# goalheart/ionic-mpnn

Measured on AMD Instinct MI355X. Metric: molecule-graph pairs/sec (fwd), batch 4096 per MI355X, higher is better.
Workload: dtype f32 (bf16x9 emulation)

## Files before the change

ionic_mpnn_amd/csrc/encoder_layout.h:

```cpp
#pragma once

#include "common.h"

namespace impnn {
namespace enc {

typedef float f32x4 __attribute__((ext_vector_type(4)));
typedef _Float16 half8 __attribute__((ext_vector_type(8)));

constexpr float kSW = 256.0f;
constexpr float kSX = 16.0f;
constexpr float kAcc = kSW * kSX;

constexpr int kD = 32;
constexpr int kKMax = 8;
constexpr int kRCap = 256;
constexpr int kECap = 1024;
constexpr int kHS = 36;
constexpr int kMsgRS = 36;
constexpr int kUpdRS = 68;
constexpr int kThreads = 1024;
constexpr int kWaves = kThreads / 64;
constexpr int kTbCapFloats = 2048;

__host__ __device__ constexpr int img_msg_floats(int K) { return K * kD * kMsgRS; }
__host__ __device__ constexpr int img_upd_floats() { return 3 * kD * kUpdRS; }
__host__ __device__ constexpr int img_vec_floats() { return 5 * kD; }
__host__ __device__ constexpr int img_floats(int K) {
  return img_msg_floats(K) + img_upd_floats() + img_vec_floats();
}
__host__ __device__ constexpr int img16_msg_halfs(int K) { return K * 2 * 2 * 512; }
__host__ __device__ constexpr int img16_upd_halfs() { return 3 * 2 * 2 * 2 * 512; }
__host__ __device__ constexpr int img16_vec_float_off(int K) { return (img16_msg_halfs(K) + img16_upd_halfs()) / 2; }
__host__ __device__ constexpr int feat_of(int q, int j) { return 16 * (j >> 2) + 4 * q + (j & 3); }
constexpr int kPf = 4;
constexpr int kImgSlot = kPf * kThreads * 4;
static_assert(kThreads == 4 * kRCap, "prologue maps 4 threads to a row");
static_assert(img_floats(kKMax) <= kImgSlot, "weight image does not fit its slot");
static_assert(img16_vec_float_off(kKMax) + img_vec_floats() <= kImgSlot, "split weight image does not fit");

constexpr int kRecRowptr = 0;
constexpr int kRecTilemax = 528;
constexpr int kRecMoloff = 544;
constexpr int kRecMolrows = 1072;
constexpr int kRecPoolrow = 1584;
constexpr int kRecRowatom = 2096;
constexpr int kEntMaxAtom = 454;
constexpr int kRecEnt = 3136;
constexpr int kRecBytes = 8192;
static_assert(kRecEnt + 4 * kECap <= kRecBytes && kRecEnt % 16 == 0, "record layout");

constexpr int kTECap = 512;
constexpr int kTECapBig = 640;
__host__ __device__ constexpr int tecap_of(int E) { return E > kTECap ? kTECapBig : kTECap; }
constexpr int kTVbMax = 256;
constexpr int kTHS = 36;
constexpr int kTAS = 32;
constexpr int kTRecRowdeg = 0;
constexpr int kTRecTilemax = 528;
constexpr int kTRecMoloff = 544;
constexpr int kTRecMolrows = 1072;
constexpr int kTRecPoolrow = 1584;
constexpr int kTRecRowatom = 2096;
constexpr int kTRecCounts = 3120;
constexpr int kTRecJdptr = 3136;
constexpr int kTRecNrun = 3664;
constexpr int kTRecGrp = 3712;
constexpr int kTRunTarget = 32;
__host__ __device__ constexpr int tgrp_cap(int Vb, int ecap) { return ecap / 4 + (Vb < kTVbMax ? Vb : kTVbMax); }
__host__ __device__ constexpr int trec_runs_off(int Vb, int ecap) { return kTRecGrp + 16 * tgrp_cap(Vb, ecap); }
__host__ __device__ constexpr int trec_used_bytes(int Vb, int ecap) {
  return (trec_runs_off(Vb, ecap) + 2 * (Vb + 2 + kTRunTarget) + 15) & ~15;
}
constexpr int kTRecBytes = 12288;
constexpr int kTRecPart1 = 8192;
__host__ __device__ constexpr int trec_lds_bytes(int Vb, int ecap) { return trec_used_bytes(Vb, ecap); }
static_assert(kTRecGrp % 16 == 0 && trec_used_bytes(kTVbMax, kTECapBig) <= kTRecBytes, "typed record layout");
__host__ __device__ constexpr int tmsg_floats(int ecap) { return (ecap + 2) * kD; }
__host__ __device__ constexpr int tmsg_off(int s, int u) { return s * kD + ((u ^ ((s >> 1) & 7)) << 2); }
__host__ __device__ constexpr int tmsg_key(int s) { return s * kD + (((s >> 1) & 7) << 2); }
static_assert(tmsg_key(kTECapBig + 1) < 65536, "message keys travel as 16 bits");
constexpr int kTUpdBlocks = 24;
constexpr int kTVecFloatOff = kTUpdBlocks * 256;
constexpr int kTUpdFloats = kTVecFloatOff + 5 * kD;
constexpr int kTUpdSlot = 2 * kThreads * 4;
constexpr int kTUpdLds = 6400;
static_assert(kTUpdFloats <= kTUpdLds && kTUpdLds <= kTUpdSlot, "typed update image");
constexpr int kXUpdHalfs = 3 * 2 * 2 * 3 * 512;
constexpr int kXVecFloatOff = kXUpdHalfs / 2;
constexpr int kXUpdFloats = kXVecFloatOff + 5 * kD;
constexpr int kXUpdSlot = 3 * kThreads * 4;
constexpr int kXUpdLds = 9472;
static_assert(kXUpdFloats <= kXUpdLds && kXUpdLds <= kXUpdSlot, "x3 update image");
constexpr int kTMatFloats = kD * kD;
inline size_t typed_prepared_floats(int S, int Vb, bool x3 = false) {
  const size_t s = S > 0 ? S : 1;
  return s * (x3 ? kXUpdSlot : kTUpdSlot) + s * (size_t)Vb * kTMatFloats + (size_t)Vb * kTMatFloats;
}

constexpr int kShareCap = kECap;
inline int plan_vmin(int n_ions, int B, int vrmax, int nwg) {
  const int64_t span = 2 * (int64_t)n_ions * B * vrmax / (nwg > 0 ? nwg : 1) + vrmax;
  const int64_t v = (span + kShareCap - 2) / (kShareCap - 1);
  return (int)(v < 1 ? 1 : (v > kRCap ? kRCap : v));
}
constexpr int kMaxHops = 128;

constexpr int kPB = 16;

struct Ws {
  size_t img_off, rows_off, vr_off, partial_off, share_off, nsub_off, desc_off, rec_off, total;
  int nwg;
  int max_sub;
  int nblk;
  int rec_bytes;
};

inline size_t align_up(size_t x, size_t a) { return (x + a - 1) / a * a; }

__host__ __device__ constexpr int tvr_of_edges(int edges, int ecap) { return (edges * kRCap + ecap - 1) / ecap; }

inline int vr_max_of(int N, int E, bool typed = false) {
  int v = typed ? (E > 4 * kTECapBig ? kRCap + 1 : tvr_of_edges(E, tecap_of(E))) : (E + 3) / 4;
  int m = N > v ? N : v;
  m = m < 1 ? 1 : m;
  return typed && m > kRCap ? kRCap : m;
}

struct PlanHeader {
  int32_t magic, kind, n_ions, B, N, E, nwg, max_sub;
  int32_t overflow;
};
constexpr int32_t kPlanMagic = 0x696d706e;
constexpr int32_t kPlanBadBit = 1 << 30;

inline Ws ws_layout(int n_ions, int B, int N, int E, int S, int Vb, int nwg, bool typed, bool x3 = false) {
  Ws w{};
  const int vrmax = vr_max_of(N, E, typed);
  w.rec_bytes = typed ? kTRecBytes : kRecBytes;
  const int win = kRCap - vrmax + 1;
  w.nwg = nwg;
  w.nblk = (B + kPB - 1) / kPB;
  const int64_t share_rows = (2 * (int64_t)n_ions * B * vrmax) / nwg + vrmax;
  const int64_t by_win = win >= 1 ? share_rows / win + 2 : (int64_t)1 << 40;
  const int64_t by_pairs = 2 * share_rows / (kRCap + 1) + 2;
  w.max_sub = (int)(by_win < by_pairs ? by_win : by_pairs);
  size_t off = 256;
  w.img_off = off;
  off = align_up(off + (typed ? (size_t)n_ions * typed_prepared_floats(S, Vb, x3)
                              : (size_t)n_ions * (S > 0 ? S : 1) * kImgSlot) * sizeof(float), 256);
  w.rows_off = off;
  off = align_up(off + (size_t)n_ions * B * sizeof(int32_t), 256);
  w.vr_off = off;
  off = align_up(off + (size_t)n_ions * B * sizeof(int32_t), 256);
  w.partial_off = off;
  off = align_up(off + (size_t)n_ions * w.nblk * sizeof(int32_t), 256);
  w.share_off = off;
  off = align_up(off + (size_t)nwg * 4 * sizeof(int32_t), 256);
  w.nsub_off = off;
  off = align_up(off + (size_t)nwg * sizeof(int32_t), 256);
// ... 101 lines not shown
```

ionic_mpnn_amd/csrc/encoder_plan.hip:

```cpp
#include "encoder_layout.h"

namespace impnn {
namespace enc {

namespace {

__global__ __launch_bounds__(64 * kPB) void plan_stats_kernel(PlanParams p) {
  __shared__ int vsum[kPB], vbad[kPB];
  __builtin_amdgcn_s_setprio(3);
  const int lane = threadIdx.x & 63, wv = threadIdx.x >> 6;
  const int g = blockIdx.x / p.nblk, blk = blockIdx.x - g * p.nblk;
  const int b = blk * kPB + wv;
  const bool have = b < p.B;
  const int64_t item = (int64_t)g * p.B + (have ? b : 0);
  int my_vr = 0, my_bad = 0;
  if (have) {
  const int32_t* ids = p.atom_ids[g] + (int64_t)b * p.N;
  const int32_t* cn = p.conn[g] + (int64_t)b * p.E * 2;
  const int32_t* bd = p.bond_ids[g] + (int64_t)b * p.E;
  int rmax = 0, cnt = 0;
  const int id_first = lane < p.N ? ids[lane] : 0;
  int emax = 0;
  for (int e0 = 0; e0 < p.E; e0 += 256) {
    int2 st[4];
// ... 798 lines not shown
        if (ce >= E) { ce -= E; ++cm; }
        const int mo = moloff[m < M ? m : 0];
        row[k] = mo + (ok ? sst[k0 + k].y : 0);
        srw[k] = mo + (ok ? sst[k0 + k].x : 0);
      }
#pragma unroll
      for (int k = 0; k < 3; ++k) {
        const bool ok = (okm >> (k0 + k)) & 1u;
        tk[k] = atomicAdd(&cnt[ok ? row[k] : kRCap + lane], 1);
        atomicAdd(&thist[ok ? sbid[k0 + k] : kTVbMax + lane], 1);
      }
#pragma unroll
      for (int k = 0; k < 3; ++k) {
        const bool ok = (okm >> (k0 + k)) & 1u;
        if (ok && tk[k] < kTick) tick[row[k] * kTick + tk[k]] = (uint16_t)es[k];
        if (ok) {
          if (pos < kTECapBig)
            elist[pos] = make_uint2((uint32_t)row[k] | ((uint32_t)srw[k] << 8) | ((uint32_t)sbid[k0 + k] << 16), (uint32_t)es[k]);
          ++pos;
        }
      }
    }
  }
  for (int s0 = kSC * kRCap; s0 < n_slots; s0 += kRCap) {
    const int slot = s0 + tid;
    int2 st = make_int2(0, 0);
    int bid = -1;
    if (slot < n_slots) {
      st = *reinterpret_cast<const int2*>(conn_c + 2 * (int64_t)slot);
      bid = bond_c[slot];
    }
    const bool ok = edge_valid(st.x, st.y, bid, N, p.Vb);
    const int m = fast_div(slot, E, rE), e = slot - m * E;
    const int mo = moloff[m < M ? m : 0];
    const int row = mo + (ok ? st.y : 0);
    int tk = kTick;
    if (ok) {
      tk = atomicAdd(&cnt[row], 1);
      atomicAdd(&thist[bid], 1);
    }
    const unsigned long long okb = __ballot(ok);
    int pos0 = 0;
    if (okb != 0ull) {
      if (lane == (int)__builtin_ctzll(okb)) pos0 = atomicAdd(&misc[1], (int)__builtin_popcountll(okb));
      pos0 = __builtin_amdgcn_readlane(pos0, (int)__builtin_ctzll(okb));
    }
    if (tk < kTick) tick[row * kTick + tk] = (uint16_t)e;
    const int pos = pos0 + (int)__builtin_popcountll(okb & ((1ull << lane) - 1));
    if (ok && pos < kTECapBig)
      elist[pos] = make_uint2((uint32_t)row | ((uint32_t)(mo + st.x) << 8) | ((uint32_t)bid << 16), (uint32_t)e);
  }
  lds_barrier();
  CSTAMP(3);

  const int my_deg = cnt[tid];
  const int dcl = my_deg > 255 ? 255 : my_deg;
  if (tid < R) {
    if (my_deg > 255) p.header->overflow = 1;
    atomicAdd(&dbins[255 - dcl], 1);
  }
  lds_barrier();
  CSTAMP(4);

  if (wave == 0) {
    const int4 h = reinterpret_cast<const int4*>(dbins)[lane];
    const int s4 = h.x + h.y + h.z + h.w;
    const int ex = wave_incl_scan(s4) - s4;
    reinterpret_cast<int4*>(dstart)[lane] = make_int4(ex, ex + h.x, ex + h.x + h.y, ex + h.x + h.y + h.z);
    __builtin_amdgcn_s_waitcnt(0xc07f);
    const int4 s = reinterpret_cast<const int4*>(dstart)[63 - lane];
    const int t4 = s.x + s.y + s.z + s.w;
    const int incl = wave_incl_scan(t4);
    const int jx = incl - t4;
    reinterpret_cast<int4*>(jdp)[lane] = make_int4(jx, jx + s.w, jx + s.w + s.z, jx + s.w + s.z + s.y);
    if (lane == 63) { jdp[kRCap] = incl; jdp[kRCap + 1] = incl; }
  } else if (wave == 1) {
    const int4 n = reinterpret_cast<const int4*>(thist)[lane];
    const int4 ng = make_int4((n.x + 3) >> 2, (n.y + 3) >> 2, (n.z + 3) >> 2, (n.w + 3) >> 2);
    const int s4 = ng.x + ng.y + ng.z + ng.w;
    const int incl = wave_incl_scan(s4);
    const int ex = incl - s4;
    reinterpret_cast<int4*>(tgb)[lane] = make_int4(ex, ex + ng.x, ex + ng.x + ng.y, ex + ng.x + ng.y + ng.z);
    const int ngrp_all = __builtin_amdgcn_readlane(incl, 63);
    int gmax = (ngrp_all + kTRunTarget - 1) / kTRunTarget;
    gmax = gmax < 2 ? 2 : gmax;
    const float rgm = 1.0f / (float)gmax;
    const int4 nr = make_int4(fast_div(ng.x + gmax - 1, gmax, rgm), fast_div(ng.y + gmax - 1, gmax, rgm),
                              fast_div(ng.z + gmax - 1, gmax, rgm), fast_div(ng.w + gmax - 1, gmax, rgm));
    const int r4 = nr.x + nr.y + nr.z + nr.w;
    const int rincl = wave_incl_scan(r4);
    int ri = rincl - r4;
    uint16_t* runs = reinterpret_cast<uint16_t*>(rec + trec_runs_off(p.Vb, p.ecap));
    for (int i = 0; i < nr.x; ++i) runs[ri++] = (uint16_t)(ex + i * gmax);
    for (int i = 0; i < nr.y; ++i) runs[ri++] = (uint16_t)(ex + ng.x + i * gmax);
    for (int i = 0; i < nr.z; ++i) runs[ri++] = (uint16_t)(ex + ng.x + ng.y + i * gmax);
    for (int i = 0; i < nr.w; ++i) runs[ri++] = (uint16_t)(ex + ng.x + ng.y + ng.z + i * gmax);
    if (lane == 63) {
      runs[rincl] = (uint16_t)incl;
      *reinterpret_cast<uint16_t*>(rec + kTRecNrun) = (uint16_t)rincl;
      misc[0] = incl;
    }
  }
  lds_barrier();
  CSTAMP(5);

  int pos = tid;
  if (tid < R) pos = dstart[255 - dcl] + atomicAdd(&dcur[255 - dcl], 1);
  place[tid] = pos;
  {
    const int my_id = idl[tid];
    r_rowatom[pos] = my_id;
    r_poolrow[tid] = (uint16_t)(pos | (my_id > 0 ? 0x8000 : 0));
    r_rowdeg[pos] = (uint16_t)my_deg;
    if ((pos & 15) == 0) r_tilemax[pos >> 4] = (unsigned char)dcl;
    r_jd[tid] = (uint16_t)jdp[tid];
    if (tid < 2) r_jd[kRCap + tid] = (uint16_t)jdp[kRCap];
    if (pos == 0) {
      r_cw[0] = (uint16_t)misc[0];
      r_cw[1] = (uint16_t)jdp[kRCap];
      r_cw[2] = (uint16_t)dcl;
    }
  }
  {
    const int n_t = thist[tid];
    const int ng = (n_t + 3) >> 2, gb = tgb[tid];
    const uint32_t dump = (uint32_t)tmsg_key(p.ecap) * 0x10001u;
    for (int jg = 0; jg < ng; ++jg) {
      const int c = n_t - 4 * jg;
      grp[gb + jg] = make_uint4((uint32_t)tid | ((uint32_t)(c < 4 ? c : 4) << 8) | ((uint32_t)(ng - jg) << 24), 0u, dump, dump);
    }
  }
  lds_barrier();
  CSTAMP(6);

  {
    auto below = [](uint4 a, uint32_t ue) {
      return (int)(((a.x & 0xffffu) < ue) + ((a.x >> 16) < ue) + ((a.y & 0xffffu) < ue) + ((a.y >> 16) < ue) +
                   ((a.z & 0xffffu) < ue) + ((a.z >> 16) < ue) + ((a.w & 0xffffu) < ue) + ((a.w >> 16) < ue));
    };
    const int nval = misc[1] < kTECapBig ? misc[1] : kTECapBig;
    for (int i0 = 0; i0 < nval; i0 += 2 * kRCap) {
      bool ok[2];
      uint2 en[2];
      int row[2], srow[2], deg[2], ix[2], gb[2], rank[2];
      uint4 ta[2], tb[2];
#pragma unroll
      for (int k = 0; k < 2; ++k) {
        const int i = i0 + k * kRCap + tid;
        ok[k] = i < nval;
        en[k] = elist[ok[k] ? i : 0];
      }
#pragma unroll
      for (int k = 0; k < 2; ++k) {
        const int rt = (int)(en[k].x & 0xffu), bid = (int)(en[k].x >> 16);
        deg[k] = cnt[rt];
        ta[k] = reinterpret_cast<const uint4*>(tick)[2 * rt];
        tb[k] = reinterpret_cast<const uint4*>(tick)[2 * rt + 1];
        row[k] = place[rt];
        srow[k] = place[(en[k].x >> 8) & 0xffu];
        gb[k] = tgb[bid];
        ix[k] = atomicAdd(&tcur[ok[k] ? bid : kTVbMax + lane], 1);
      }
#pragma unroll
      for (int k = 0; k < 2; ++k) {
        rank[k] = below(ta[k], en[k].y) + below(tb[k], en[k].y);
        if (deg[k] > kTick) {
          const int rt = (int)(en[k].x & 0xffu);
          int lo = 0, hi = M - 1;
          while (lo < hi) {
            const int mid = (lo + hi + 1) >> 1;
            if (moloff[mid] <= rt) lo = mid; else hi = mid - 1;
          }
          const int t = rt - moloff[lo];
          const int32_t* cm = conn_c + 2 * (int64_t)lo * E;
          const int32_t* bm = bond_c + (int64_t)lo * E;
          rank[k] = 0;
          for (int e2 = 0; e2 < (int)en[k].y; ++e2) {
            const int2 s2 = *reinterpret_cast<const int2*>(cm + 2 * e2);
            rank[k] += (s2.y == t && edge_valid(s2.x, s2.y, bm[e2], N, p.Vb)) ? 1 : 0;
          }
        }
        rank[k] = jdp[rank[k] < 256 ? rank[k] : 255];
      }
#pragma unroll
      for (int k = 0; k < 2; ++k) {
        if (ok[k]) {
          unsigned char* ge = reinterpret_cast<unsigned char*>(&grp[gb[k] + (ix[k] >> 2)]);
          ge[4 + (ix[k] & 3)] = (unsigned char)srow[k];
          reinterpret_cast<uint16_t*>(ge + 8)[ix[k] & 3] = (uint16_t)tmsg_key(rank[k] + row[k]);
        }
      }
    }
  }
  lds_barrier();
  CSTAMP(9);

  {
    const int ngrp = misc[0];
    uint4* r_grp = reinterpret_cast<uint4*>(rec + kTRecGrp);
    for (int i = tid; i < ngrp; i += kRCap) r_grp[i] = grp[i];
  }
  CSTAMP(15);
  lds_barrier();
// ... 43 lines not shown
```

ionic_mpnn_amd/csrc/encoder_typed.hip:

```cpp
#include "encoder_device.h"
#include "encoder_layout.h"

namespace impnn {
namespace enc {

namespace {

constexpr int kOffUpd = 0;
constexpr int off_h(bool x3) { return kOffUpd + (x3 ? kXUpdLds : kTUpdLds); }
constexpr int kTHSBig3 = 32;
constexpr int off_msg(bool x3, int hs = kTHS) { return off_h(x3) + kRCap * hs; }
constexpr int off_rec(bool x3, int ecap, int hs = kTHS) { return off_msg(x3, hs) + tmsg_floats(ecap); }
constexpr size_t lds_fixed_bytes(bool x3, int Vb, int ecap, int hs = kTHS) {
  return sizeof(float) * (size_t)off_rec(x3, ecap, hs) + trec_lds_bytes(Vb, ecap);
}
static_assert(lds_fixed_bytes(true, kTVbMax, kTECap) <= 160 * 1024 && lds_fixed_bytes(false, kTVbMax, kTECapBig) <= 160 * 1024 &&
                  lds_fixed_bytes(true, kTVbMax, kTECapBig, kTHSBig3) <= 160 * 1024,
              "LDS budget");

typedef __bf16 bf16x8 __attribute__((ext_vector_type(8)));
struct B3 {
  bf16x8 p0, p1, p2;
};
__device__ __forceinline__ void split_pair(float x, float y, unsigned& w0, unsigned& w1, unsigned& w2) {
// ... 2 lines not shown
  const unsigned x1b = __builtin_bit_cast(unsigned, x1), y1b = __builtin_bit_cast(unsigned, y1);
  const float x2 = x1 - __builtin_bit_cast(float, x1b & 0xffff0000u), y2 = y1 - __builtin_bit_cast(float, y1b & 0xffff0000u);
  w0 = __builtin_amdgcn_perm(yb, xb, 0x07060302u);
  w1 = __builtin_amdgcn_perm(y1b, x1b, 0x07060302u);
  w2 = __builtin_amdgcn_perm(__builtin_bit_cast(unsigned, y2), __builtin_bit_cast(unsigned, x2), 0x07060302u);
}
__device__ __forceinline__ B3 split8x3(f32x4 a, f32x4 b) {
  union {
    bf16x8 v;
    unsigned u[4];
  } q0, q1, q2;
  split_pair(a[0], a[1], q0.u[0], q1.u[0], q2.u[0]);
  split_pair(a[2], a[3], q0.u[1], q1.u[1], q2.u[1]);
  split_pair(b[0], b[1], q0.u[2], q1.u[2], q2.u[2]);
  split_pair(b[2], b[3], q0.u[3], q1.u[3], q2.u[3]);
  B3 r;
  r.p0 = q0.v;
  r.p1 = q1.v;
  r.p2 = q2.v;
  return r;
}
__device__ __forceinline__ f32x4 mfmab(bf16x8 a, bf16x8 b, f32x4 c) {
  return __builtin_amdgcn_mfma_f32_16x16x32_bf16(a, b, c, 0, 0, 0);
}
__device__ __forceinline__ void mma9x2(f32x4& c0, f32x4& c1, const __bf16* blk0, const __bf16* blk1, int lane, const B3& b) {
  const bf16x8 a00 = *reinterpret_cast<const bf16x8*>(blk0 + lane * 8);
  const bf16x8 a01 = *reinterpret_cast<const bf16x8*>(blk0 + 512 + lane * 8);
  const bf16x8 a02 = *reinterpret_cast<const bf16x8*>(blk0 + 1024 + lane * 8);
  const bf16x8 a10 = *reinterpret_cast<const bf16x8*>(blk1 + lane * 8);
  const bf16x8 a11 = *reinterpret_cast<const bf16x8*>(blk1 + 512 + lane * 8);
  const bf16x8 a12 = *reinterpret_cast<const bf16x8*>(blk1 + 1024 + lane * 8);
  c0 = mfmab(a02, b.p2, c0);  c1 = mfmab(a12, b.p2, c1);
  c0 = mfmab(a01, b.p2, c0);  c1 = mfmab(a11, b.p2, c1);
  c0 = mfmab(a02, b.p1, c0);  c1 = mfmab(a12, b.p1, c1);
  c0 = mfmab(a00, b.p2, c0);  c1 = mfmab(a10, b.p2, c1);
  c0 = mfmab(a02, b.p0, c0);  c1 = mfmab(a12, b.p0, c1);
  c0 = mfmab(a01, b.p1, c0);  c1 = mfmab(a11, b.p1, c1);
  c0 = mfmab(a00, b.p1, c0);  c1 = mfmab(a10, b.p1, c1);
  c0 = mfmab(a01, b.p0, c0);  c1 = mfmab(a11, b.p0, c1);
  c0 = mfmab(a00, b.p0, c0);  c1 = mfmab(a10, b.p0, c1);
}

template <int ABID>
__device__ __forceinline__ f32x4 mfma1(float a, float b, f32x4 c) {
  return __builtin_amdgcn_mfma_f32_4x4x1f32(a, b, c, 3, ABID, 0);
}

typedef float f32x2v __attribute__((ext_vector_type(2)));
struct Grp {
  uint4 ge;
  f32x2v aq;
};
struct Run {
  f32x4 bq[4];
  Grp first;
};

#ifndef IMPNN_T_PF
#define IMPNN_T_PF 0
#endif
#ifndef IMPNN_T_EARLY
#define IMPNN_T_EARLY 0
#endif
constexpr int kPfWhere = IMPNN_T_PF, kRunsEarly = IMPNN_T_EARLY;

template <bool STAMPS, bool X3, int HS = kTHS>
__global__ __launch_bounds__(kThreads, kThreads / 256) void encoder_typed_kernel(TEncParams p) {
  extern __shared__ __align__(16) float smem[];
  constexpr int kUpdLds = X3 ? kXUpdLds : kTUpdLds, kUpdSlot = X3 ? kXUpdSlot : kTUpdSlot;
  constexpr int kNPf = X3 ? 3 : 2;
  float* const wupd = smem + kOffUpd;
  float* const wvec = wupd + (X3 ? kXVecFloatOff : kTVecFloatOff);
  float* const hbuf = smem + off_h(X3);
  float* const msg = smem + off_msg(X3, HS);
  const int zero_slot = p.ecap + 1;
  unsigned char* const recl = reinterpret_cast<unsigned char*>(smem + off_rec(X3, p.ecap, HS));
  const int rec_lds = p.rec_lds;
  float* const atab = reinterpret_cast<float*>(recl + rec_lds);
  const uint16_t* const r_rowdeg = reinterpret_cast<const uint16_t*>(recl + kTRecRowdeg);
  const unsigned char* const r_tilemax = recl + kTRecTilemax;
  const uint16_t* const r_moloff = reinterpret_cast<const uint16_t*>(recl + kTRecMoloff);
  const uint16_t* const r_molrows = reinterpret_cast<const uint16_t*>(recl + kTRecMolrows);
  const uint16_t* const r_poolrow = reinterpret_cast<const uint16_t*>(recl + kTRecPoolrow);
  const int32_t* const r_rowatom = reinterpret_cast<const int32_t*>(recl + kTRecRowatom);
  const uint16_t* const r_jdptr = reinterpret_cast<const uint16_t*>(recl + kTRecJdptr);
  const uint16_t* const r_runs = reinterpret_cast<const uint16_t*>(recl + trec_runs_off(p.Vb, p.ecap));
  int* const run_ctr = reinterpret_cast<int*>(recl + kTRecCounts + 8);
  const uint4* const r_grp = reinterpret_cast<const uint4*>(recl + kTRecGrp);

  const int tid = threadIdx.x, lane = tid & 63;
  const int wave = __builtin_amdgcn_readfirstlane(tid >> 6);
  const int a = lane & 15, q = lane >> 4;
  unsigned long long* stamp = STAMPS && p.stamps ? p.stamps + (size_t)blockIdx.x * 32 : nullptr;
  if (stamp && tid == 0) stamp[0] = __builtin_amdgcn_s_memtime();

  {
    const PlanHeader hd = *p.header;
    if (hd.magic != kPlanMagic || hd.kind != 1 || hd.nwg != (int)gridDim.x || hd.max_sub != p.max_sub ||
        hd.B != p.B || hd.n_ions != p.n_ions || hd.overflow != 0) {
      const float nan = __builtin_nanf("");
      for (int g = 0; g < p.n_ions; ++g)
        for (int64_t t = (int64_t)blockIdx.x * kThreads + tid; t < (int64_t)p.B * kD; t += (int64_t)gridDim.x * kThreads)
          p.pooled[g][t] = nan;
      return;
    }
  }
  const int c_begin = blockIdx.x * p.max_sub;
  const int c_end = c_begin + __builtin_amdgcn_readfirstlane(p.nsub[blockIdx.x]);
  if (c_begin >= c_end) return;

  if (p.atab_lds)
    for (int t = tid; t < (p.Va + 1) * (kTAS / 4); t += kThreads)
      st4(atab + 4 * t, t < p.Va * (kD / 4) ? ld4(p.atom_table + 4 * t) : f32x4{0.f, 0.f, 0.f, 0.f});
  if (tid < kD) msg[zero_slot * kD + tid] = 0.f;
  unsigned long long t_pro = 0, t_steps = 0, t_pool = 0, t_mark = 0, t_msg = 0;
  if (stamp && tid == 0) t_mark = __builtin_amdgcn_s_memtime();

  auto pool = [&](int M, int m0, int g) {
    float* out_g = p.pooled[g];
    for (int t0 = 0; t0 < M * 64; t0 += kThreads) {
      const int t = t0 + tid;
      const int part = t & 7, f4 = (t >> 3) & 7, m = t >> 6;
      f32x4 acc = {0.f, 0.f, 0.f, 0.f};
      if (m < M) {
        const int nr = r_molrows[m], mo = r_moloff[m];
        for (int n = part; n < nr; n += 8) {
          const int pr = r_poolrow[mo + n];
          if (pr & 0x8000) acc += ld4(hbuf + (pr & 0xff) * HS + 4 * f4);
        }
      }
#pragma unroll
      for (int i = 0; i < 4; ++i) {
        float v = acc[i];
        v += __builtin_bit_cast(float, __builtin_amdgcn_update_dpp(0, __builtin_bit_cast(int, v), 0xb1, 0xf, 0xf, true));
        v += __builtin_bit_cast(float, __builtin_amdgcn_update_dpp(0, __builtin_bit_cast(int, v), 0x4e, 0xf, 0xf, true));
        v += __builtin_bit_cast(float, __builtin_amdgcn_update_dpp(0, __builtin_bit_cast(int, v), 0x141, 0xf, 0xf, true));
        acc[i] = v;
      }
      if (m < M && part == 0) st4(out_g + (int64_t)(m0 + m) * kD + 4 * f4, acc);
    }
  };
  auto fill_h0 = [&]() {
    const int row = tid >> 2, sub = tid & 3;
    const int id = r_rowatom[row];
    f32x4 v0 = {0.f, 0.f, 0.f, 0.f}, v1 = v0;
    if ((unsigned)id < (unsigned)p.Va) {
      if (p.atab_lds) {
        v0 = ld4(atab + id * kTAS + 8 * sub);
        v1 = ld4(atab + id * kTAS + 8 * sub + 4);
      } else {
        v0 = ld4(p.atom_table + (int64_t)id * kD + 8 * sub);
        v1 = ld4(p.atom_table + (int64_t)id * kD + 8 * sub + 4);
      }
    }
    st4(hbuf + row * HS + 8 * sub, v0);
    st4(hbuf + row * HS + 8 * sub + 4, v1);
  };

  if (p.S == 0) {
    for (int c = c_begin; c < c_end; ++c) {
      const unsigned char* rc = p.rec + (size_t)c * kTRecBytes;
      if (8 * tid < rec_lds) reinterpret_cast<uint2*>(recl)[tid] = reinterpret_cast<const uint2*>(rc)[tid];
      const int4 dsc = reinterpret_cast<const int4*>(p.desc)[c];
      lds_barrier();
      fill_h0();
      lds_barrier();
      pool(__builtin_amdgcn_readfirstlane(dsc.y), __builtin_amdgcn_readfirstlane(dsc.x),
           __builtin_amdgcn_readfirstlane(dsc.w) >> 16);
      lds_barrier();
    }
    return;
  }

  const bool rec_big = rec_lds > kTRecPart1;
  const unsigned char* rec_c = p.rec + (size_t)c_begin * kTRecBytes;
  uint2 rec_n8 = reinterpret_cast<const uint2*>(rec_c)[tid];
  uint32_t rec_n4 = rec_big ? reinterpret_cast<const uint32_t*>(rec_c + kTRecPart1)[tid] : 0u;
  int4 dsc_next = reinterpret_cast<const int4*>(p.desc)[c_begin];

  const uint32_t* const grp_x = reinterpret_cast<const uint32_t*>(r_grp);
  const int kh = lane >> 5, f = lane & 31;
  const int boff = kh * 512 + f * 4;
  const int ysh = 8 * (lane & 3), zsh = 16 * kh;
  const int acol = 16 * kh + 2 * ((lane >> 2) & 7);

  for (int c = c_begin; c < c_end; ++c) {
    const int4 dsc = dsc_next;
    const int m0 = __builtin_amdgcn_readfirstlane(dsc.x), M = __builtin_amdgcn_readfirstlane(dsc.y);
    const int rg = __builtin_amdgcn_readfirstlane(dsc.w);
    const int R = rg & 0xffff, g = rg >> 16;
    const int ntiles = (R + 15) >> 4;
    const float* upd_g = p.upd[g];
    const float* tmat_g = p.tmat[g];
    if (8 * tid < rec_lds) reinterpret_cast<uint2*>(recl)[tid] = rec_n8;
    if (rec_big && kTRecPart1 + 4 * tid < rec_lds) reinterpret_cast<uint32_t*>(recl + kTRecPart1)[tid] = rec_n4;
    {
      const int cn = (c + 1) < c_end ? (c + 1) : c;
      const unsigned char* rn = p.rec + (size_t)cn * kTRecBytes;
      rec_n8 = reinterpret_cast<const uint2*>(rn)[tid];
      if (rec_big) rec_n4 = reinterpret_cast<const uint32_t*>(rn + kTRecPart1)[tid];
      dsc_next = reinterpret_cast<const int4*>(p.desc)[cn];
    }
    lds_barrier();
    fill_h0();
    if (tid == 0) *run_ctr = 2 * kWaves;
    lds_barrier();
    if (stamp && tid == 0) {
      const unsigned long long t = __builtin_amdgcn_s_memtime();
      t_pro += t - t_mark;
      t_mark = t;
    }
    const int nrun = __builtin_amdgcn_readfirstlane(*reinterpret_cast<const uint16_t*>(recl + kTRecNrun));

    Run P, Q;
    int gP = 0, nP = 0, gQ = 0, nQ = 0;
    bool haveP = false, haveQ = false;
    const bool sP = wave < nrun, sQ = wave + kWaves < nrun;
    const int sgP = __builtin_amdgcn_readfirstlane(r_runs[sP ? wave : 0]);
    const int snP = __builtin_amdgcn_readfirstlane(r_runs[(sP ? wave : 0) + 1]) - sgP;
    const int sgQ = __builtin_amdgcn_readfirstlane(r_runs[sQ ? wave + kWaves : 0]);
    const int snQ = __builtin_amdgcn_readfirstlane(r_runs[(sQ ? wave + kWaves : 0) + 1]) - sgQ;
    const int soP = sP ? (__builtin_amdgcn_readfirstlane(grp_x[4 * sgP]) & 0xff) * kTMatFloats : 0;
    const int soQ = sQ ? (__builtin_amdgcn_readfirstlane(grp_x[4 * sgQ]) & 0xff) * kTMatFloats : 0;
    const int lboffP = sP ? boff : 0, lboffQ = sQ ? boff : 0;
    f32x4 pf[kNPf];
    auto fetch_pf = [&](int s_) {
#pragma unroll
      for (int i = 0; i < kNPf; ++i) pf[i] = ld4(upd_g + (int64_t)s_ * kUpdSlot + 4 * (tid + i * kThreads));
    };
    auto fetch_P = [&](int s_) {
      const float* tm = tmat_g + (size_t)s_ * p.Vb * kTMatFloats;
#pragma unroll
      for (int i = 0; i < 4; ++i) P.bq[i] = ld4(tm + soP + lboffP + i * 128);
    };
    auto fetch_Q = [&](int s_) {
      const float* tm = tmat_g + (size_t)s_ * p.Vb * kTMatFloats;
#pragma unroll
      for (int i = 0; i < 4; ++i) Q.bq[i] = ld4(tm + soQ + lboffQ + i * 128);
    };
    if (kPfWhere != 0) fetch_pf(0);
    if (kRunsEarly >= 1) fetch_P(0);
    if (kRunsEarly >= 2) fetch_Q(0);
    for (int s = 0; s < p.S; ++s) {
      const float* tm_s = tmat_g + (size_t)s * p.Vb * kTMatFloats;
      __builtin_amdgcn_s_setprio(2);
      {
        const float* const abase = hbuf + acol;
        auto load_group = [&](int e, Grp& G) {
          G.ge = r_grp[e];
          const int src = __builtin_amdgcn_ubfe(G.ge.y, ysh, 8);
          G.aq = *reinterpret_cast<const f32x2v*>(abase + src * HS);
        };
        auto compute = [&](const Grp& G, const f32x4 (&bq)[4]) {
          f32x4 acc0 = {0.f, 0.f, 0.f, 0.f}, acc1 = acc0;
#ifndef IMPNN_DIAG_NO_MSG_MFMA
          acc0 = mfma1<0>(G.aq[0], bq[0][0], acc0);
          acc1 = mfma1<0>(G.aq[1], bq[0][1], acc1);
          acc0 = mfma1<1>(G.aq[0], bq[0][2], acc0);
          acc1 = mfma1<1>(G.aq[1], bq[0][3], acc1);
          acc0 = mfma1<2>(G.aq[0], bq[1][0], acc0);
          acc1 = mfma1<2>(G.aq[1], bq[1][1], acc1);
          acc0 = mfma1<3>(G.aq[0], bq[1][2], acc0);
          acc1 = mfma1<3>(G.aq[1], bq[1][3], acc1);
          acc0 = mfma1<4>(G.aq[0], bq[2][0], acc0);
          acc1 = mfma1<4>(G.aq[1], bq[2][1], acc1);
          acc0 = mfma1<5>(G.aq[0], bq[2][2], acc0);
          acc1 = mfma1<5>(G.aq[1], bq[2][3], acc1);
          acc0 = mfma1<6>(G.aq[0], bq[3][0], acc0);
          acc1 = mfma1<6>(G.aq[1], bq[3][1], acc1);
          acc0 = mfma1<7>(G.aq[0], bq[3][2], acc0);
          acc1 = mfma1<7>(G.aq[1], bq[3][3], acc1);
#else
          acc0[0] = G.aq[0] + bq[0][0] + bq[3][3];
          acc1[1] = G.aq[1] + bq[1][1] + bq[2][2];
#endif
          float x0 = acc0[0] + acc1[0], x1 = acc0[1] + acc1[1], x2 = acc0[2] + acc1[2], x3 = acc0[3] + acc1[3];
          asm volatile("s_nop 1\n\tv_permlane32_swap_b32 %0, %1\n\tv_permlane32_swap_b32 %2, %3"
                       : "+v"(x0), "+v"(x1), "+v"(x2), "+v"(x3));
          msg[__builtin_amdgcn_ubfe(G.ge.z, zsh, 16) ^ f] = x0 + x1;
          msg[__builtin_amdgcn_ubfe(G.ge.w, zsh, 16) ^ f] = x2 + x3;
        };
        auto run_type = [&](int g_, int n_, Run& Rn) {
          const int end = g_ + n_;
          Grp T;
          int e = g_;
          while (true) {
            if (e + 1 < end) load_group(e + 1, T);
            compute(Rn.first, Rn.bq);
            if (++e >= end) break;
            if (e + 1 < end) load_group(e + 1, Rn.first);
            compute(T, Rn.bq);
            if (++e >= end) break;
          }
        };
        auto fetch = [&](bool have, int r, int& g_, int& n_, Run& Rn, const float* tm) {
          const int rc = have ? r : 0;
          g_ = __builtin_amdgcn_readfirstlane(r_runs[rc]);
          n_ = __builtin_amdgcn_readfirstlane(r_runs[rc + 1]) - g_;
          const int type = have ? (__builtin_amdgcn_readfirstlane(grp_x[4 * g_]) & 0xff) : 0;
          const float* bp = tm + (size_t)type * kTMatFloats + (have ? boff : 0);
#pragma unroll
          for (int i = 0; i < 4; ++i) Rn.bq[i] = ld4(bp + i * 128);
        };
        auto next_run = [&]() {
          int r = 0;
          if (lane == 0) r = atomicAdd(run_ctr, 1);
          return __builtin_amdgcn_readfirstlane(r);
        };
        auto take = [&](int r, int& g_, int& n_, Run& Rn) {
          fetch(true, r, g_, n_, Rn, tm_s);
          load_group(g_, Rn.first);
        };
        auto landed = [](f32x4 (&b)[4]) {
          asm volatile("" : "+v"(b[0]), "+v"(b[1]), "+v"(b[2]), "+v"(b[3]) : : "memory");
        };
        if (kPfWhere == 0) fetch_pf(s);
        if (kRunsEarly < 1) fetch_P(s);
        if (kRunsEarly < 2) fetch_Q(s);
        haveP = sP; gP = sgP; nP = snP;
        haveQ = sQ; gQ = sgQ; nQ = snQ;
        if (haveP) load_group(gP, P.first);
        if (haveQ) load_group(gQ, Q.first);
        if (haveP) {
          if (!haveQ) {
            landed(P.bq);
            run_type(gP, nP, P);
          } else {
            while (true) {
              landed(P.bq);
              run_type(gP, nP, P);
              const int rP = next_run();
              if (rP >= nrun) {
                landed(Q.bq);
                run_type(gQ, nQ, Q);
                break;
              }
              take(rP, gP, nP, P);
              landed(Q.bq);
              run_type(gQ, nQ, Q);
              const int rQ = next_run();
              if (rQ >= nrun) {
                landed(P.bq);
                run_type(gP, nP, P);
                break;
              }
              take(rQ, gQ, nQ, Q);
            }
          }
        }
      }
#pragma unroll
      for (int i = 0; i < kNPf; ++i)
        if (4 * (tid + i * kThreads) < kUpdLds) st4(wupd + 4 * (tid + i * kThreads), pf[i]);
      const bool mstamp = stamp && c == c_begin && s == 1;
      if (mstamp && lane == 0) stamp[16 + wave] = __builtin_amdgcn_s_memtime();
      lds_barrier();
      if (tid == 0) *run_ctr = 2 * kWaves;
      if (mstamp && tid == 0) stamp[12] = __builtin_amdgcn_s_memtime();
      if (stamp && tid == 0 && c == c_begin && s == 1) t_msg = __builtin_amdgcn_s_memtime();

      int my_tile = -1;
      {
        const int grp = wave & 3, slot = wave >> 2, q4 = ntiles >> 2, r4 = ntiles & 3;
        const int heavy = (4 - r4) * q4;
        if (grp >= r4) {
          if (slot < q4) my_tile = slot * (4 - r4) + (grp - r4);
        } else if (slot <= q4) {
          my_tile = heavy + slot * r4 + grp;
        }
      }
      const bool has_tile = my_tile >= 0 && my_tile < ntiles;
      if (has_tile) {
        const int tile = my_tile;
        const int row = tile * 16 + a;
        const int deg = r_rowdeg[row];
        const int maxdeg = __builtin_amdgcn_readfirstlane(r_tilemax[tile]);
        f32x4 agg0 = {0.f, 0.f, 0.f, 0.f}, agg1 = agg0;
        for (int d0 = 0; d0 < maxdeg; d0 += 4) {
          const uint2 jd = *reinterpret_cast<const uint2*>(r_jdptr + d0);
          int sl[4];
          sl[0] = d0 + 0 < deg ? (int)(jd.x & 0xffffu) + row : zero_slot;
          sl[1] = d0 + 1 < deg ? (int)(jd.x >> 16) + row : zero_slot;
          sl[2] = d0 + 2 < deg ? (int)(jd.y & 0xffffu) + row : zero_slot;
          sl[3] = d0 + 3 < deg ? (int)(jd.y >> 16) + row : zero_slot;
          f32x4 m0v[4], m1v[4];
#pragma unroll
          for (int j = 0; j < 4; ++j) {
            const int o = tmsg_off(sl[j], q);
            m0v[j] = ld4(msg + o);
            m1v[j] = ld4(msg + (o ^ 16));
          }
#pragma unroll
          for (int j = 0; j < 4; ++j) {
// ... 219 lines not shown
```

Baseline: 35.36 million.

## Pack run entries with type and length, drop rowatom from LDS, pipeline records

Run descriptors become 32-bit entries holding the first group, the matrix type (which doubles as the matrix offset) and the run length. This removes the extra LDS reads of the next run start and of the group header when fetching a run. The row-atom section is no longer copied into LDS; each thread prefetches its atom id from global memory alongside the next record, and the LDS record shrinks by that cut. The run counter is now initialised in the planner, one barrier is removed from the record handoff, and pooling is changed to one molecule per wave with batched loads. The trade-off is tighter bit-field limits, which are checked by static asserts.

```diff
diff --git a/ionic_mpnn_amd/csrc/encoder_layout.h b/ionic_mpnn_amd/csrc/encoder_layout.h
--- a/ionic_mpnn_amd/csrc/encoder_layout.h
+++ b/ionic_mpnn_amd/csrc/encoder_layout.h
@@ -68,14 +68,33 @@
 constexpr int kTRecGrp = 3712;
 constexpr int kTRunTarget = 32;
 __host__ __device__ constexpr int tgrp_cap(int Vb, int ecap) { return ecap / 4 + (Vb < kTVbMax ? Vb : kTVbMax); }
+constexpr int kTRunGrpBits = 10, kTRunTypeBits = 8;
+constexpr uint32_t kTRunGrpMask = (1u << kTRunGrpBits) - 1u;
+constexpr uint32_t kTRunMatMask = ((1u << kTRunTypeBits) - 1u) << kTRunGrpBits;
+constexpr int kTRunLenShift = kTRunGrpBits + kTRunTypeBits;
+__host__ __device__ constexpr int trun_gmax(int groups) {
+  return (groups + kTRunTarget - 1) / kTRunTarget < 2 ? 2 : (groups + kTRunTarget - 1) / kTRunTarget;
+}
+__host__ __device__ constexpr uint32_t trun_entry(int first, int type, int groups) {
+  return (uint32_t)first | ((uint32_t)type << kTRunGrpBits) | ((uint32_t)groups << kTRunLenShift);
+}
+static_assert(tgrp_cap(kTVbMax, kTECapBig) <= (1 << kTRunGrpBits) && kTVbMax <= (1 << kTRunTypeBits) &&
+                  trun_gmax(tgrp_cap(kTVbMax, kTECapBig)) < (1 << (32 - kTRunLenShift)) &&
+                  (1 << kTRunGrpBits) == kD * kD,
+              "run entry fields (the type field doubles as the matrix offset: kTMatFloats = 1 << kTRunGrpBits)");
 __host__ __device__ constexpr int trec_runs_off(int Vb, int ecap) { return kTRecGrp + 16 * tgrp_cap(Vb, ecap); }
 __host__ __device__ constexpr int trec_used_bytes(int Vb, int ecap) {
-  return (trec_runs_off(Vb, ecap) + 2 * (Vb + 2 + kTRunTarget) + 15) & ~15;
+  return (trec_runs_off(Vb, ecap) + 4 * ((Vb < kTVbMax ? Vb : kTVbMax) + kTRunTarget) + 15) & ~15;
 }
 constexpr int kTRecBytes = 12288;
 constexpr int kTRecPart1 = 8192;
-__host__ __device__ constexpr int trec_lds_bytes(int Vb, int ecap) { return trec_used_bytes(Vb, ecap); }
+constexpr int kTRecCut = 4 * kRCap;
+__host__ __device__ constexpr int trec_lds_off(int off) { return off < kTRecRowatom ? off : off - kTRecCut; }
+__host__ __device__ constexpr int trec_lds_bytes(int Vb, int ecap) { return trec_used_bytes(Vb, ecap) - kTRecCut; }
 static_assert(kTRecGrp % 16 == 0 && trec_used_bytes(kTVbMax, kTECapBig) <= kTRecBytes, "typed record layout");
+static_assert(kTRecRowatom % 8 == 0 && kTRecCut % 16 == 0 && kTRecRowatom + kTRecCut <= kTRecCounts &&
+                  kTRecPart1 > kTRecRowatom + kTRecCut,
+              "the cut is a whole number of the copy's 8-byte words, inside the first part of the copy");
 __host__ __device__ constexpr int tmsg_floats(int ecap) { return (ecap + 2) * kD; }
 __host__ __device__ constexpr int tmsg_off(int s, int u) { return s * kD + ((u ^ ((s >> 1) & 7)) << 2); }
 __host__ __device__ constexpr int tmsg_key(int s) { return s * kD + (((s >> 1) & 7) << 2); }
diff --git a/ionic_mpnn_amd/csrc/encoder_plan.hip b/ionic_mpnn_amd/csrc/encoder_plan.hip
--- a/ionic_mpnn_amd/csrc/encoder_plan.hip
+++ b/ionic_mpnn_amd/csrc/encoder_plan.hip
@@ -904,21 +904,25 @@
     const int ex = incl - s4;
     reinterpret_cast<int4*>(tgb)[lane] = make_int4(ex, ex + ng.x, ex + ng.x + ng.y, ex + ng.x + ng.y + ng.z);
     const int ngrp_all = __builtin_amdgcn_readlane(incl, 63);
-    int gmax = (ngrp_all + kTRunTarget - 1) / kTRunTarget;
-    gmax = gmax < 2 ? 2 : gmax;
+    const int gmax = trun_gmax(ngrp_all);
     const float rgm = 1.0f / (float)gmax;
     const int4 nr = make_int4(fast_div(ng.x + gmax - 1, gmax, rgm), fast_div(ng.y + gmax - 1, gmax, rgm),
                               fast_div(ng.z + gmax - 1, gmax, rgm), fast_div(ng.w + gmax - 1, gmax, rgm));
     const int r4 = nr.x + nr.y + nr.z + nr.w;
     const int rincl = wave_incl_scan(r4);
     int ri = rincl - r4;
-    uint16_t* runs = reinterpret_cast<uint16_t*>(rec + trec_runs_off(p.Vb, p.ecap));
-    for (int i = 0; i < nr.x; ++i) runs[ri++] = (uint16_t)(ex + i * gmax);
-    for (int i = 0; i < nr.y; ++i) runs[ri++] = (uint16_t)(ex + ng.x + i * gmax);
-    for (int i = 0; i < nr.z; ++i) runs[ri++] = (uint16_t)(ex + ng.x + ng.y + i * gmax);
-    for (int i = 0; i < nr.w; ++i) runs[ri++] = (uint16_t)(ex + ng.x + ng.y + ng.z + i * gmax);
+    uint32_t* runs = reinterpret_cast<uint32_t*>(rec + trec_runs_off(p.Vb, p.ecap));
+    auto put_runs = [&](int type, int first, int groups, int n) {
+      for (int i = 0; i < n; ++i) {
+        const int left = groups - i * gmax;
+        runs[ri++] = trun_entry(first + i * gmax, type, left < gmax ? left : gmax);
+      }
+    };
+    put_runs(4 * lane + 0, ex, ng.x, nr.x);
+    put_runs(4 * lane + 1, ex + ng.x, ng.y, nr.y);
+    put_runs(4 * lane + 2, ex + ng.x + ng.y, ng.z, nr.z);
+    put_runs(4 * lane + 3, ex + ng.x + ng.y + ng.z, ng.w, nr.w);
     if (lane == 63) {
-      runs[rincl] = (uint16_t)incl;
       *reinterpret_cast<uint16_t*>(rec + kTRecNrun) = (uint16_t)rincl;
       misc[0] = incl;
     }
@@ -941,6 +945,7 @@
       r_cw[0] = (uint16_t)misc[0];
       r_cw[1] = (uint16_t)jdp[kRCap];
       r_cw[2] = (uint16_t)dcl;
+      *reinterpret_cast<int32_t*>(rec + kTRecCounts + 8) = 2 * kWaves;
     }
   }
   {
diff --git a/ionic_mpnn_amd/csrc/encoder_typed.hip b/ionic_mpnn_amd/csrc/encoder_typed.hip
--- a/ionic_mpnn_amd/csrc/encoder_typed.hip
+++ b/ionic_mpnn_amd/csrc/encoder_typed.hip
@@ -108,11 +108,10 @@
   const uint16_t* const r_moloff = reinterpret_cast<const uint16_t*>(recl + kTRecMoloff);
   const uint16_t* const r_molrows = reinterpret_cast<const uint16_t*>(recl + kTRecMolrows);
   const uint16_t* const r_poolrow = reinterpret_cast<const uint16_t*>(recl + kTRecPoolrow);
-  const int32_t* const r_rowatom = reinterpret_cast<const int32_t*>(recl + kTRecRowatom);
-  const uint16_t* const r_jdptr = reinterpret_cast<const uint16_t*>(recl + kTRecJdptr);
-  const uint16_t* const r_runs = reinterpret_cast<const uint16_t*>(recl + trec_runs_off(p.Vb, p.ecap));
-  int* const run_ctr = reinterpret_cast<int*>(recl + kTRecCounts + 8);
-  const uint4* const r_grp = reinterpret_cast<const uint4*>(recl + kTRecGrp);
+  const uint16_t* const r_jdptr = reinterpret_cast<const uint16_t*>(recl + trec_lds_off(kTRecJdptr));
+  const uint32_t* const r_runs = reinterpret_cast<const uint32_t*>(recl + trec_lds_off(trec_runs_off(p.Vb, p.ecap)));
+  int* const run_ctr = reinterpret_cast<int*>(recl + trec_lds_off(kTRecCounts + 8));
+  const uint4* const r_grp = reinterpret_cast<const uint4*>(recl + trec_lds_off(kTRecGrp));
 
   const int tid = threadIdx.x, lane = tid & 63;
   const int wave = __builtin_amdgcn_readfirstlane(tid >> 6);
@@ -142,17 +141,24 @@
   unsigned long long t_pro = 0, t_steps = 0, t_pool = 0, t_mark = 0, t_msg = 0;
   if (stamp && tid == 0) t_mark = __builtin_amdgcn_s_memtime();
 
+  constexpr int kPoolBatch = 8;
   auto pool = [&](int M, int m0, int g) {
     float* out_g = p.pooled[g];
-    for (int t0 = 0; t0 < M * 64; t0 += kThreads) {
-      const int t = t0 + tid;
-      const int part = t & 7, f4 = (t >> 3) & 7, m = t >> 6;
+    const int part = tid & 7, f4 = (tid >> 3) & 7;
+    for (int m = wave; m < M; m += kWaves) {
+      const int nr = __builtin_amdgcn_readfirstlane(r_molrows[m]), mo = __builtin_amdgcn_readfirstlane(r_moloff[m]);
       f32x4 acc = {0.f, 0.f, 0.f, 0.f};
-      if (m < M) {
-        const int nr = r_molrows[m], mo = r_moloff[m];
-        for (int n = part; n < nr; n += 8) {
-          const int pr = r_poolrow[mo + n];
-          if (pr & 0x8000) acc += ld4(hbuf + (pr & 0xff) * HS + 4 * f4);
+      for (int n0 = part; n0 - part < nr; n0 += 8 * kPoolBatch) {
+        int pr[kPoolBatch];
+        f32x4 hv[kPoolBatch];
+#pragma unroll
+        for (int i = 0; i < kPoolBatch; ++i) pr[i] = r_poolrow[mo + (n0 + 8 * i < nr ? n0 + 8 * i : 0)];
+#pragma unroll
+        for (int i = 0; i < kPoolBatch; ++i) hv[i] = ld4(hbuf + (pr[i] & 0xff) * HS + 4 * f4);
+#pragma unroll
+        for (int i = 0; i < kPoolBatch; ++i) {
+          const f32x4 sum = acc + hv[i];
+          if (n0 + 8 * i < nr && (pr[i] & 0x8000)) acc = sum;
         }
       }
 #pragma unroll
@@ -163,12 +169,11 @@
         v += __builtin_bit_cast(float, __builtin_amdgcn_update_dpp(0, __builtin_bit_cast(int, v), 0x141, 0xf, 0xf, true));
         acc[i] = v;
       }
-      if (m < M && part == 0) st4(out_g + (int64_t)(m0 + m) * kD + 4 * f4, acc);
+      if (part == 0) st4(out_g + (int64_t)(m0 + m) * kD + 4 * f4, acc);
     }
   };
-  auto fill_h0 = [&]() {
-    const int row = tid >> 2, sub = tid & 3;
-    const int id = r_rowatom[row];
+  auto fill_h0 = [&](int id, int t) {
+    const int row = t >> 2, sub = t & 3;
     f32x4 v0 = {0.f, 0.f, 0.f, 0.f}, v1 = v0;
     if ((unsigned)id < (unsigned)p.Va) {
       if (p.atab_lds) {
@@ -183,71 +188,74 @@
     st4(hbuf + row * HS + 8 * sub + 4, v1);
   };
 
+  const int rec_used = rec_lds + kTRecCut;
+  const bool rec_big = rec_used > kTRecPart1;
+  uint2 rec_n8;
+  uint32_t rec_n4 = 0u;
+  int dsc_next, aid_next;
+  auto load_record = [&](int cn, int t) {
+    const unsigned char* rn = p.rec + (size_t)cn * kTRecBytes;
+    rec_n8 = reinterpret_cast<const uint2*>(rn)[t];
+    if (rec_big) rec_n4 = reinterpret_cast<const uint32_t*>(rn + kTRecPart1)[t];
+    aid_next = reinterpret_cast<const int32_t*>(rn + kTRecRowatom)[t >> 2];
+    dsc_next = p.desc[4 * cn + (t & 3)];
+  };
+  auto take_record = [&](int c) {
+    const int aid = aid_next;
+    int t = tid;
+    asm volatile("" : "+v"(t));
+    if (8 * t < rec_used && (8 * t < kTRecRowatom || 8 * t >= kTRecRowatom + kTRecCut))
+      *reinterpret_cast<uint2*>(recl + trec_lds_off(8 * t)) = rec_n8;
+    if (rec_big && kTRecPart1 + 4 * t < rec_used)
+      reinterpret_cast<uint32_t*>(recl + trec_lds_off(kTRecPart1))[t] = rec_n4;
+    fill_h0(aid, t);
+    load_record((c + 1) < c_end ? (c + 1) : c, t);
+    lds_barrier();
+  };
+  load_record(c_begin, tid);
+  lds_barrier();
+
   if (p.S == 0) {
     for (int c = c_begin; c < c_end; ++c) {
-      const unsigned char* rc = p.rec + (size_t)c * kTRecBytes;
-      if (8 * tid < rec_lds) reinterpret_cast<uint2*>(recl)[tid] = reinterpret_cast<const uint2*>(rc)[tid];
-      const int4 dsc = reinterpret_cast<const int4*>(p.desc)[c];
-      lds_barrier();
-      fill_h0();
-      lds_barrier();
-      pool(__builtin_amdgcn_readfirstlane(dsc.y), __builtin_amdgcn_readfirstlane(dsc.x),
-           __builtin_amdgcn_readfirstlane(dsc.w) >> 16);
+      const int m0 = __builtin_amdgcn_readlane(dsc_next, 0), M = __builtin_amdgcn_readlane(dsc_next, 1);
+      const int g = __builtin_amdgcn_readlane(dsc_next, 3) >> 16;
+      take_record(c);
+      pool(M, m0, g);
       lds_barrier();
     }
     return;
   }
 
-  const bool rec_big = rec_lds > kTRecPart1;
-  const unsigned char* rec_c = p.rec + (size_t)c_begin * kTRecBytes;
-  uint2 rec_n8 = reinterpret_cast<const uint2*>(rec_c)[tid];
-  uint32_t rec_n4 = rec_big ? reinterpret_cast<const uint32_t*>(rec_c + kTRecPart1)[tid] : 0u;
-  int4 dsc_next = reinterpret_cast<const int4*>(p.desc)[c_begin];
-
-  const uint32_t* const grp_x = reinterpret_cast<const uint32_t*>(r_grp);
   const int kh = lane >> 5, f = lane & 31;
   const int boff = kh * 512 + f * 4;
   const int ysh = 8 * (lane & 3), zsh = 16 * kh;
   const int acol = 16 * kh + 2 * ((lane >> 2) & 7);
 
   for (int c = c_begin; c < c_end; ++c) {
-    const int4 dsc = dsc_next;
-    const int m0 = __builtin_amdgcn_readfirstlane(dsc.x), M = __builtin_amdgcn_readfirstlane(dsc.y);
-    const int rg = __builtin_amdgcn_readfirstlane(dsc.w);
+    const int m0 = __builtin_amdgcn_readlane(dsc_next, 0), M = __builtin_amdgcn_readlane(dsc_next, 1);
+    const int rg = __builtin_amdgcn_readlane(dsc_next, 3);
     const int R = rg & 0xffff, g = rg >> 16;
     const int ntiles = (R + 15) >> 4;
     const float* upd_g = p.upd[g];
     const float* tmat_g = p.tmat[g];
-    if (8 * tid < rec_lds) reinterpret_cast<uint2*>(recl)[tid] = rec_n8;
-    if (rec_big && kTRecPart1 + 4 * tid < rec_lds) reinterpret_cast<uint32_t*>(recl + kTRecPart1)[tid] = rec_n4;
-    {
-      const int cn = (c + 1) < c_end ? (c + 1) : c;
-      const unsigned char* rn = p.rec + (size_t)cn * kTRecBytes;
-      rec_n8 = reinterpret_cast<const uint2*>(rn)[tid];
-      if (rec_big) rec_n4 = reinterpret_cast<const uint32_t*>(rn + kTRecPart1)[tid];
-      dsc_next = reinterpret_cast<const int4*>(p.desc)[cn];
-    }
-    lds_barrier();
-    fill_h0();
-    if (tid == 0) *run_ctr = 2 * kWaves;
-    lds_barrier();
+    take_record(c);
     if (stamp && tid == 0) {
       const unsigned long long t = __builtin_amdgcn_s_memtime();
       t_pro += t - t_mark;
       t_mark = t;
     }
-    const int nrun = __builtin_amdgcn_readfirstlane(*reinterpret_cast<const uint16_t*>(recl + kTRecNrun));
+    const int nrun = __builtin_amdgcn_readfirstlane(*reinterpret_cast<const uint16_t*>(recl + trec_lds_off(kTRecNrun)));
 
     Run P, Q;
     int gP = 0, nP = 0, gQ = 0, nQ = 0;
     bool haveP = false, haveQ = false;
     const bool sP = wave < nrun, sQ = wave + kWaves < nrun;
-    const int sgP = __builtin_amdgcn_readfirstlane(r_runs[sP ? wave : 0]);
-    const int snP = __builtin_amdgcn_readfirstlane(r_runs[(sP ? wave : 0) + 1]) - sgP;
-    const int sgQ = __builtin_amdgcn_readfirstlane(r_runs[sQ ? wave + kWaves : 0]);
-    const int snQ = __builtin_amdgcn_readfirstlane(r_runs[(sQ ? wave + kWaves : 0) + 1]) - sgQ;
-    const int soP = sP ? (__builtin_amdgcn_readfirstlane(grp_x[4 * sgP]) & 0xff) * kTMatFloats : 0;
-    const int soQ = sQ ? (__builtin_amdgcn_readfirstlane(grp_x[4 * sgQ]) & 0xff) * kTMatFloats : 0;
+    const uint32_t seP = __builtin_amdgcn_readfirstlane(r_runs[sP ? wave : 0]);
+    const uint32_t seQ = __builtin_amdgcn_readfirstlane(r_runs[sQ ? wave + kWaves : 0]);
+    const int sgP = seP & kTRunGrpMask, snP = seP >> kTRunLenShift;
+    const int sgQ = seQ & kTRunGrpMask, snQ = seQ >> kTRunLenShift;
+    const int soP = sP ? (int)(seP & kTRunMatMask) : 0;
+    const int soQ = sQ ? (int)(seQ & kTRunMatMask) : 0;
     const int lboffP = sP ? boff : 0, lboffQ = sQ ? boff : 0;
     f32x4 pf[kNPf];
     auto fetch_pf = [&](int s_) {
@@ -319,12 +327,11 @@
             if (++e >= end) break;
           }
         };
-        auto fetch = [&](bool have, int r, int& g_, int& n_, Run& Rn, const float* tm) {
-          const int rc = have ? r : 0;
-          g_ = __builtin_amdgcn_readfirstlane(r_runs[rc]);
-          n_ = __builtin_amdgcn_readfirstlane(r_runs[rc + 1]) - g_;
-          const int type = have ? (__builtin_amdgcn_readfirstlane(grp_x[4 * g_]) & 0xff) : 0;
-          const float* bp = tm + (size_t)type * kTMatFloats + (have ? boff : 0);
+        auto fetch = [&](int r, int& g_, int& n_, Run& Rn, const float* tm) {
+          const uint32_t en = __builtin_amdgcn_readfirstlane(r_runs[r]);
+          g_ = en & kTRunGrpMask;
+          n_ = en >> kTRunLenShift;
+          const float* bp = tm + (en & kTRunMatMask) + boff;
 #pragma unroll
           for (int i = 0; i < 4; ++i) Rn.bq[i] = ld4(bp + i * 128);
         };
@@ -334,7 +341,7 @@
           return __builtin_amdgcn_readfirstlane(r);
         };
         auto take = [&](int r, int& g_, int& n_, Run& Rn) {
-          fetch(true, r, g_, n_, Rn, tm_s);
+          fetch(r, g_, n_, Rn, tm_s);
           load_group(g_, Rn.first);
         };
         auto landed = [](f32x4 (&b)[4]) {
```

New measurement: 35.15 million. No clear change (-0.6%).
